# kkoutini/PaSST

Measured on AMD Instinct MI355X. Metric: clips/s (10s@32k) fwd+bwd passt_s, higher is better.
Workload: dtype bf16; 1 GPU; passt_s_swa_p16_128_ap476 train step (mel front end + mixup + fwd + BCE + bwd + adamw), 768/12/12, 474 tokens (s_patchout_t=40,f=4), random-init weights; global_batch=64, per_gpu_batch=64, parallelism=dp1, gemm_launch=persistent, 256 workgroups, input=waveform (B,1,320000) f32 resident in HBM

## Files before the change

### include/passt_amd.h

```cpp
#ifndef PASST_AMD_H
#define PASST_AMD_H

#include <stdint.h>

#ifdef __cplusplus
extern "C" {
#endif

#define PA_ABI_VERSION 6

enum { PA_F32 = 0, PA_BF16 = 1 };

enum {
    PA_OK = 0,
    PA_EINVAL = -1,
    PA_EUNSUPPORTED = -2,
    PA_ELAUNCH = -3,
    PA_ECOMM = -4
};

int pa_abi_version(void);
const char* pa_error_string(int code);
const char* pa_last_hip_error(void);

// ... 103 lines not shown
    int32_t ldolp;
    void* out_lp2;
    int32_t ldolp2;
    int32_t split_k;
    int32_t tune;
    float* colsum_out;
    float* colsum_ws;
    int32_t colsum_accumulate;
    int32_t reserved;
    int32_t colscale_n;
    float colscale;
} pa_gemm_args;
#define PA_GEMM_BLOCKED_PRE 0x100
#define PA_GEMM_NO_PERSIST 0x400
#define PA_GEMM_EPILOGUE_V3 0x1000
#define PA_GEMM_COLSUM_DEFER 0x2000
int pa_gemm_blocked_pre_ok(int M, int N, int K);
int64_t pa_gemm_blocked_pre_elems(int M, int N);
int64_t pa_gemm_colsum_ws_floats(int M, int N);
int pa_gemm_nt(const pa_gemm_args* a, void* stream);
int pa_gemm_nt_splitk_plan(int M, int N, int K, int epilogue, int dtype);
int64_t pa_gemm_nt_splitk_ws_floats(int M, int N, int K, int epilogue, int dtype);
int pa_gemm_nt_splitk(const pa_gemm_args* a, float* ws, int64_t ws_floats, void* stream);
int pa_gemm_nt_rowscale(const pa_gemm_args* a, const float* rowscale, void* stream);
int pa_gemm_nt_splitk_rowscale(const pa_gemm_args* a, const float* rowscale, float* ws, int64_t ws_floats, void* stream);
int pa_gemm_tn(const pa_gemm_args* a, void* stream);
#define PA_TN_BATCH_MAX 4
#ifndef PA_TN_STEP_ROWS
#define PA_TN_STEP_ROWS 48
#endif
int pa_gemm_tn_step_rows(void);
int pa_gemm_tn_batched(const pa_gemm_args* a, int n, void* stream);
int pa_gemm_tn_batched_plan(const pa_gemm_args* a, int n, int n_long, int long_steps, void* stream);
int pa_gather_rows(const void* in, const int32_t* idx, int n_idx, int64_t row_bytes, void* out, void* stream);
int pa_scatter_rows(const void* in, const int32_t* idx, int n_idx, int64_t row_bytes, void* out, void* stream);
int pa_tail_inject(const float* rows, const int32_t* idx, int n_idx, const float* add0, const float* add1, float* dx,
                   void* dx_lp, int dtype, int M, int D, void* stream);
int pa_zero2d(void* ptr, int64_t pitch_bytes, int64_t width_bytes, int64_t rows, void* stream);
int pa_reduce_partials(const float* partial, int splits, int64_t n, float* out, int accumulate,
                       void* stream);
#define PA_REDUCE_BATCH_MAX 12
#define PA_REDUCE_SLABS 0
#define PA_REDUCE_ROWS 1
typedef struct pa_reduce_desc {
    const float* partial;
    float* out;
    int64_t n;
    int32_t splits;
    int32_t accumulate;
    int64_t pitch;
    int32_t mode;
    int32_t reserved;
} pa_reduce_desc;
int pa_reduce_partials_batched(const pa_reduce_desc* d, int n, void* stream);
int pa_gemm_last_colsum_rows(void);
int pa_rowsum(const void* in, int dtype, int R, int C, int ld, float* out, int accumulate,
              void* stream);
int64_t pa_colsum_ws_floats(int R, int C);
int pa_colsum(const void* in, int dtype, int R, int C, int ld, float* out, int accumulate, float* ws,
              void* stream);
int pa_colsum_f32(const float* in, int R, int C, int ld, float* out, int accumulate, void* stream);

#define PA_ATTN_Q_PRESCALED 1
#define PA_ATTN_BWD_TWO_PASS 2
#define PA_ATTN_BWD_SINGLE_PASS 4
#define PA_ATTN_BWD_SINGLE_PASS_W16 8
// ... 138 lines not shown
```

### passt_amd/_lib.py

```python
import ctypes as C
import os

_HERE = os.path.dirname(os.path.abspath(__file__))
LIB_PATH = os.path.join(_HERE, "libpasst_amd.so")
LIB_PATH = os.environ.get("PASST_AMD_LIB", LIB_PATH)

PA_F32, PA_BF16 = 0, 1
EPI_STORE, EPI_GELU, EPI_RESID, EPI_DGELU, EPI_PARTIAL = 0, 1, 2, 3, 4

vp, i32, i64, f32 = C.c_void_p, C.c_int32, C.c_int64, C.c_float


class MelParams(C.Structure):
    _fields_ = [("n_fft", i32), ("hop", i32), ("n_mels", i32), ("n_frames", i32),
                ("preemph", f32), ("mel_low", f32), ("inv_mel_delta", f32), ("log_eps", f32),
                ("out_add", f32), ("out_scale", f32),
                ("fmask_start", i32), ("fmask_end", i32), ("tmask_start", i32), ("tmask_end", i32)]


class MelClipParams(C.Structure):
    _fields_ = [("mel_low", f32), ("inv_mel_delta", f32),
                ("fmask_start", i32), ("fmask_end", i32), ("tmask_start", i32), ("tmask_end", i32)]


# ... 29 lines not shown
    "pa_mel_frontend_fwd_varlen": (i32, [vp, i32, i32, vp, vp, vp, vp, vp, i32, f32, C.POINTER(MelParams), vp]),
    "pa_mel_frontend_bwd": (i32, [vp, i32, i32, vp, vp, vp, vp, vp, vp, i64, C.POINTER(MelParams), vp]),
    "pa_mel_frontend_bwd_varlen": (i32, [vp, i32, i32, vp, vp, vp, vp, vp, i32, vp, vp, i64, C.POINTER(MelParams), vp]),
    "pa_mel_frontend_fwd_varlen_aug": (i32, [vp, i32, i32, vp, vp, vp, vp, vp, i32, f32, C.POINTER(MelParams), vp, vp]),
    "pa_mel_frontend_bwd_varlen_aug": (i32, [vp, i32, i32, vp, vp, vp, vp, vp, i32, vp, vp, i64, C.POINTER(MelParams), vp, vp]),
    "pa_convert_f32": (i32, [vp, vp, i64, i32, vp]),
    "pa_convert_f32_rowscale": (i32, [vp, vp, vp, i32, i32, i32, vp]),
    "pa_convert_to_f32": (i32, [vp, i32, vp, i64, vp]),
    "pa_transpose": (i32, [vp, i32, i32, i32, i32, vp, i32, i32, vp]),
    "pa_stage_weights": (i32, [vp, i32, i32, i32, vp]),
    "pa_layernorm_fwd": (i32, [vp, vp, vp, vp, i32, vp, vp, i32, i32, f32, vp]),
    "pa_layernorm_bwd_ws_floats": (i64, [i32, i32]),
    "pa_layernorm_bwd": (i32, [vp, i32, vp, vp, vp, vp, vp, vp, vp, vp, vp, vp, i32, vp, i32, i32, vp]),
    "pa_layernorm_bwd_rows": (i32, [i32]),
    "pa_layernorm_bwd_partial": (i32, [vp, i32, vp, vp, vp, vp, vp, vp, vp, vp, i32, i32, vp]),
    "pa_layernorm_bwd2": (i32, [vp, i32, vp, vp, vp, vp, vp, vp, vp, vp, vp, vp, vp, i32, vp, i32, i32, vp]),
    "pa_layernorm_bwd2_partial": (i32, [vp, i32, vp, vp, vp, vp, vp, vp, vp, vp, vp, i32, i32, vp]),
    "pa_layernorm_bwd_rowscale": (i32, [vp, i32, vp, vp, vp, vp, vp, vp, vp, vp, vp, vp, vp, vp, i32, vp, i32, i32, vp]),
    "pa_layernorm_bwd_partial_rowscale": (i32, [vp, i32, vp, vp, vp, vp, vp, vp, vp, vp, vp, vp, i32, i32, vp]),
    "pa_tail_inject": (i32, [vp, vp, i32, vp, vp, vp, vp, i32, i32, i32, vp]),
    "pa_gemm_last_colsum_rows": (i32, []),
    "pa_gemm_colsum_ws_floats": (i64, [i32, i32]),
    "pa_gemm_blocked_pre_ok": (i32, [i32, i32, i32]),
    "pa_gemm_blocked_pre_elems": (i64, [i32, i32]),
    "pa_gemm_nt": (i32, [C.POINTER(GemmArgs), vp]),
    "pa_gemm_nt_splitk_plan": (i32, [i32, i32, i32, i32, i32]),
    "pa_gemm_nt_splitk_ws_floats": (i64, [i32, i32, i32, i32, i32]),
    "pa_gemm_nt_splitk": (i32, [C.POINTER(GemmArgs), vp, i64, vp]),
    "pa_gemm_nt_rowscale": (i32, [C.POINTER(GemmArgs), vp, vp]),
    "pa_gemm_nt_splitk_rowscale": (i32, [C.POINTER(GemmArgs), vp, vp, i64, vp]),
    "pa_gemm_tn": (i32, [C.POINTER(GemmArgs), vp]),
    "pa_gemm_tn_batched": (i32, [C.POINTER(GemmArgs), i32, vp]),
    "pa_gemm_tn_batched_plan": (i32, [C.POINTER(GemmArgs), i32, i32, i32, vp]),
    "pa_gemm_tn_step_rows": (i32, []),
    "pa_reduce_partials_batched": (i32, [C.POINTER(ReduceDesc), i32, vp]),
    "pa_colsum_ws_floats": (i64, [i32, i32]),
    "pa_colsum": (i32, [vp, i32, i32, i32, i32, vp, i32, vp, vp]),
    "pa_reduce_partials": (i32, [vp, i32, i64, vp, i32, vp]),
    "pa_rowsum": (i32, [vp, i32, i32, i32, i32, vp, i32, vp]),
    "pa_colsum_f32": (i32, [vp, i32, i32, i32, vp, i32, vp]),
    "pa_attention_fwd": (i32, [vp, i32, vp, i32, vp, i32, i32, i32, i32, f32, i32, i32, vp]),
    "pa_attention_fwd_varlen": (i32, [vp, i32, vp, i32, vp, vp, i32, i32, i32, i32, f32, i32, i32, vp]),
    "pa_attention_probs": (i32, [vp, i32, vp, vp, vp, vp, i32, i32, i32, i32, i32, f32, i32, i32, vp]),
    "pa_attention_probs_grad": (i32, [vp, i32, vp, vp, i32, i32, vp, vp, vp, i32, i32, i32, i32, i32, i32, f32, i32, i32, vp]),
    "pa_attention_rollout_ws_floats": (i64, [i64, i32, i32, i32, i32, i32]),
    "pa_attention_rollout": (i32, [vp, i32, vp, vp, i32, i32, vp, vp, vp, vp, i64, i32, i32, i32, i32, i32, i32, i32, f32, f32, f32, f32,
                                   i32, i32, vp]),
    "pa_attention_bwd_ws_floats": (i64, [i32, i32, i32]),
    "pa_attention_bwd": (i32, [vp, i32, vp, vp, i32, vp, vp, vp, i32, i32, i32, i32, i32, f32, i32, i32, vp]),
    "pa_attention_bwd_varlen_ws_floats": (i64, [i64, i32, i32, i32]),
    "pa_attention_bwd_varlen": (i32, [vp, i32, vp, vp, i32, vp, vp, vp, i32, vp, i32, i32, i32, i32, f32, i32, i32, vp]),
    "pa_gather_rows": (i32, [vp, vp, i32, i64, vp, vp]),
    "pa_scatter_rows": (i32, [vp, vp, i32, i64, vp, vp]),
    "pa_zero2d": (i32, [vp, i64, i64, i64, vp]),
    "pa_patch_gather": (i32, [vp, i32, i32, i32, vp, vp, i32, i32, i32, i32, vp, i32, vp]),
    "pa_patch_pos_table": (i32, [vp, vp, i32, vp, i32, vp, vp, i32, i32, i32, vp, vp, vp, vp, vp, i32, i32, vp]),
    "pa_patch_gather_varlen": (i32, [vp, i32, i32, i32, vp, vp, vp, i32, i32, i32, i32, vp, i32, vp]),
    "pa_patch_pos_table_varlen": (i32, [vp, vp, i32, vp, i32, vp, vp, i32, i32, vp, vp, vp, vp, vp]),
    "pa_patch_input_bwd_varlen": (i32, [vp, i32, vp, i32, i32, i32, i32, i32, i32, vp, vp]),
    "pa_patch_bwd_varlen": (i32, [vp, i32, i32, vp, i32, i32, i32, vp, vp, vp, vp, vp, vp, i32, vp]),
    "pa_patch_input_bwd_rows": (i32, [vp, i32, i32, vp, i32, i32, i32, i32, i32, i32, i32, vp, vp]),
    "pa_patch_bwd_rows": (i32, [vp, i32, i32, vp, vp, vp, i32, i32, i32, i32, vp, vp, vp, vp, vp, vp, i32, vp]),
    "pa_patch_bwd": (i32, [vp, i32, i32, i32, vp, vp, i32, i32, i32, i32, vp, vp, vp, vp, vp, vp, vp, i32, vp, i32, vp]),
    "pa_patch_input_bwd_ws_ints": (i64, [i32, i32, i32, i32, i32]),
    "pa_patch_input_bwd": (i32, [vp, i32, i32, i32, vp, vp, i32, i32, i32, i32, i32, vp, vp, vp]),
    "pa_head_pre_fwd": (i32, [vp, i32, i32, i32, vp, vp, f32, vp, vp, f32, vp, vp, vp, vp]),
# ... 104 lines not shown
```

### passt_amd/csrc/gemm.hip

```cpp
#include <algorithm>
#include <cstring>
#include <type_traits>

#include "pa_mma.h"

namespace pa {

static constexpr int NT_GROUP_M = 4;
static constexpr int BM = 128, BN = 128, KB = 128;
static constexpr int TILE_BYTES = BM * KB;
static constexpr int GEMM_LDS = 2 * 2 * TILE_BYTES;

#ifdef PA_PROBE
__device__ unsigned long long* g_probe_buf = nullptr;
static constexpr int PROBE_SLOTS = 512;
#define PA_PROBE_STAMP(cond, idx)                                                                             \
    do {                                                                                                      \
        if ((cond) && (wave & 3) == 0 && lane == 0 && (idx) < PROBE_SLOTS)                                    \
            ((unsigned long long*)(smem + G::LDS))[(wave >> 2) * PROBE_SLOTS + (idx)] = __builtin_amdgcn_s_memtime(); \
    } while (0)
#define PA_PROBE_FLAG(a, bit) (((a).reserved >> (bit)) & 1)
#define PA_PROBE_STAMP_TN(cond, idx)                                                                          \
    do {                                                                                                      \
        if ((cond) && (wave & 3) == 0 && lane == 0 && (idx) < PROBE_SLOTS)                                    \
            ((unsigned long long*)(smem + TN_LDS))[(wave >> 2) * PROBE_SLOTS + (idx)] = __builtin_amdgcn_s_memtime(); \
    } while (0)
#else
#define PA_PROBE_STAMP(cond, idx) do {} while (0)
#define PA_PROBE_STAMP_TN(cond, idx) do {} while (0)
#define PA_PROBE_FLAG(a, bit) 0
#endif


static constexpr int SLAB_BYTES = 32 * 68 * 4;

static int finish_gemm_colsum(const pa_gemm_args& a, int rows, hipStream_t st);

template <int EPI, int TM> __host__ __device__ constexpr int aux_depth() {
    return EPI == PA_EPI_DGELU ? TM : (EPI == PA_EPI_RESID ? (TM <= 3 ? TM : 2) : 0);
}

template <int EPI>
__device__ __forceinline__ void load_bias8(const pa_gemm_args& a, int n0, int wc, int lane, float (&bias8)[8]) {
    const int ncol = n0 + wc * 64 + (lane & 7) * 8;
#pragma unroll
    for (int e = 0; e < 8; ++e) bias8[e] = 0.f;
    if constexpr (EPI != PA_EPI_PARTIAL && EPI != PA_EPI_DGELU) {
        if (a.bias && ncol < a.N) {
            const f32x4 lo = *(const f32x4*)(a.bias + ncol), hi = *(const f32x4*)(a.bias + ncol + 4);
#pragma unroll
            for (int e = 0; e < 4; ++e) { bias8[e] = lo[e]; bias8[4 + e] = hi[e]; }
        }
    }
}

template <typename T, int EPI, int TM = 2, bool RS = false>
__device__ __forceinline__ void gemm_epilogue(const pa_gemm_args& a, f32x16 (&acc)[TM][2], float* slab, int m0,
                                              int n0, int split, int wr, int wc, int lane, const float (&bias8)[8],
                                              int colsum_row = 0, const float* rowscale = nullptr) {
    static_assert(!RS || EPI == PA_EPI_RESID, "row factors: the residual epilogue only");
    const int erow = lane >> 3, ecol = (lane & 7) * 8;
    const int ncol = n0 + wc * 64 + ecol;
    const bool colok = ncol < a.N;
// ... 1385 lines not shown
            }
#pragma unroll
            for (int i = 0; i < 2; ++i)
#pragma unroll
                for (int j = 0; j < 2; ++j) mma32<T>(acc[i][j], fa[i], fb[j]);
        }
    }
    __syncthreads();
    const float nobias[8] = {0.f, 0.f, 0.f, 0.f, 0.f, 0.f, 0.f, 0.f};
    gemm_epilogue<T, PA_EPI_PARTIAL, 2>(a, acc, (float*)(smem + wave * SLAB_BYTES), m0, n0, blockIdx.y, wr, wc, lane, nobias);
}

__device__ __forceinline__ int tn2_swz(int row, int c) { return row * 512 + ((c ^ ((row & 3) << 2)) << 4); }

__device__ __forceinline__ bf16x8 tn2_frag(const char* tile, int ms, int cbase, int lane) {
    const int p = lane & 15, g = (lane >> 4) & 1, h = lane >> 5;
    const int r1 = ms * 16 + h * 8 + (p >> 2);
    const int col = cbase + g * 16 + (p & 3) * 4;
    const int within = (col & 7) * 2;
    const bf16x4 lo = lds_tr16(tile + tn2_swz(r1, col >> 3) + within);
    const bf16x4 hi = lds_tr16(tile + tn2_swz(r1 + 4, col >> 3) + within);
    bf16x8 f;
    f[0] = lo[0]; f[1] = lo[1]; f[2] = lo[2]; f[3] = lo[3];
    f[4] = hi[0]; f[5] = hi[1]; f[6] = hi[2]; f[7] = hi[3];
    return f;
}

static constexpr int TN_ROWS = PA_TN_STEP_ROWS;
static constexpr int TN_STAGES = 3;
static constexpr int TN_OP_BYTES = TN_ROWS * 512, TN_STAGE_BYTES = 2 * TN_OP_BYTES;
static constexpr int TN_LDS = TN_STAGES * TN_STAGE_BYTES;
static_assert(TN_ROWS % 16 == 0 && TN_ROWS * 512 % (8 * 1024) == 0, "whole 16-token phases, whole 1 KiB pieces per wave");

__device__ __forceinline__ void gemm_tn_stagger_range(const pa_gemm_args& a, const int tiles_n, const int tile_id, const int st_begin,
                                                      const int nsteps, float* out, const int ldo, float* cs_out) {
    const bool CSUM = cs_out != nullptr && tile_id % tiles_n == 0;
    constexpr int TM = 4, WN = 4, MROWS = TN_ROWS, NPH = MROWS / 16;
    constexpr int OP_BYTES = TN_OP_BYTES, STAGE_BYTES = TN_STAGE_BYTES;
    constexpr int PER = OP_BYTES / 1024 / 8;
    extern __shared__ __attribute__((aligned(16))) char smem[];
    const int tid = threadIdx.x;
    const int lane = tid & 63;
    const int wave = __builtin_amdgcn_readfirstlane(tid >> 6);
    const int wr = wave / WN, wc = wave % WN;
    const int bid = tile_id;
    const int m0 = (bid / tiles_n) * 256, n0 = (bid % tiles_n) * 256;
    const int Mtok = a.K;

    uint32_t voffA[PER], voffB[PER];
    int rowin[PER];
#pragma unroll
    for (int i = 0; i < PER; ++i) {
        const int q = wave * PER + i;
        const int row = q * 2 + (lane >> 5);
        const int pc = lane & 31;
        const int c = pc ^ ((row & 3) << 2);
        rowin[i] = row;
        voffA[i] = (uint32_t)row * (uint32_t)a.lda * 2u + (uint32_t)min(m0 + c * 8, a.M - 8) * 2u;
        voffB[i] = (uint32_t)row * (uint32_t)a.ldb * 2u + (uint32_t)min(n0 + c * 8, a.N - 8) * 2u;
    }
    const char* baseA = (const char*)a.A + (int64_t)st_begin * MROWS * a.lda * 2;
    const char* baseB = (const char*)a.B + (int64_t)st_begin * MROWS * a.ldb * 2;
    auto dma = [&](const bool opB, const char* base, int ld, const uint32_t (&voff)[PER], char* dst, int step) __attribute__((always_inline)) {
        const char* sb = base + (int64_t)step * MROWS * ld * 2;
        const int valid = Mtok - (st_begin + step) * MROWS;
        if (valid >= MROWS) {
            if (opB) {
#pragma unroll
// ... 122 lines not shown
#pragma unroll
                    for (int j = 0; j < 2; ++j) mma32_first<bf16>(acc[i][j], fa[i], fb[j]);
            } else {
#pragma unroll
                for (int i = 0; i < TM; ++i)
#pragma unroll
                    for (int j = 0; j < 2; ++j) mma32<bf16>(acc[i][j], fa[i], fb[j]);
            }
            if (CSUM) asm volatile("s_nop 1\n\tv_mfma_f32_32x32x16_bf16 %0, %1, %2, %0" : "+v"(accb) : "v"(fcs), "v"(ones));
            __builtin_amdgcn_s_setprio(0);
            PA_PROBE_STAMP_TN(t >= 4 && t < 12, ((t - 4) * NPH + ph) * 4 + 2);
            if (ph == NPH - 1 && wr == 0) {
                wait_stage();
                asm volatile("s_waitcnt lgkmcnt(0)" ::: "memory");
            }
            __builtin_amdgcn_sched_barrier(0);
            __builtin_amdgcn_s_barrier();
            PA_PROBE_STAMP_TN(t >= 4 && t < 12, ((t - 4) * NPH + ph) * 4 + 3);
        };
        phase(std::integral_constant<int, 0>{});
        phase(std::integral_constant<int, 1>{});
        phase(std::integral_constant<int, 2>{});
        if constexpr (NPH == 4) phase(std::integral_constant<int, 3>{});
        static_assert(NPH == 3 || NPH == 4, "three or four 16-token phases per stage");
        slot = slot1;
    }
    if (wr == 0) __builtin_amdgcn_s_barrier();
#ifdef PA_PROBE
    __syncthreads();
    if (g_probe_buf && blockIdx.x < 8)
        for (int i = tid; i < 2 * PROBE_SLOTS; i += 512)
            g_probe_buf[(size_t)blockIdx.x * 2 * PROBE_SLOTS + i] = ((unsigned long long*)(smem + TN_LDS))[i];
#endif
    {
        pa_gemm_args e = a;
        e.out_f32 = out;
        e.ldo32 = ldo;
        gemm_epilogue_f32_direct<PA_EPI_PARTIAL, TM>(e, acc, nullptr, m0, n0, 0, wr, wc, lane);
    }
    if (CSUM) {
        if ((lane & 31) == 0) {
            float* dst = cs_out;
#pragma unroll
            for (int r = 0; r < 16; ++r) {
                const int m = m0 + wr * 128 + wc * 32 + acc_row(r, lane);
                if (m < a.M) dst[m] = accb[r];
            }
        }
    }
}

__device__ __forceinline__ void gemm_tn_stagger_item(const pa_gemm_args& a, const int tiles_n, const int tile_id, const int split,
                                                     const int steps_per_split) {
    const int steps_total = (a.K + TN_ROWS - 1) / TN_ROWS;
    const int st_begin = split * steps_per_split;
    const int nsteps = min(steps_total, st_begin + steps_per_split) - st_begin;
    gemm_tn_stagger_range(a, tiles_n, tile_id, st_begin, nsteps, a.out_f32 + (int64_t)split * a.M * a.ldo32, a.ldo32,
                          a.colsum_ws ? a.colsum_ws + (int64_t)split * a.M : nullptr);
}

__global__ __launch_bounds__(512) void gemm_tn_stagger_kernel(const pa_gemm_args a, const int tiles_n, const int nwg,
                                                              const int steps_per_split) {
    gemm_tn_stagger_item(a, tiles_n, xcd_swizzle(blockIdx.x, nwg), blockIdx.y, steps_per_split);
}

struct TnBatch {
    pa_gemm_args a[PA_TN_BATCH_MAX];
    int32_t first[PA_TN_BATCH_MAX + 1];
    int32_t tiles_n[PA_TN_BATCH_MAX], nwg[PA_TN_BATCH_MAX], per[PA_TN_BATCH_MAX];
    int32_t tfirst[PA_TN_BATCH_MAX + 1];
    int32_t n, order;
};
__global__ __launch_bounds__(512) void gemm_tn_stagger_batched_kernel(const TnBatch b) {
    int p = 0, t, split;
    if (b.order == 1) {
        const int logical = xcd_swizzle(blockIdx.x, b.first[b.n]);
        const int tiles_all = b.tfirst[b.n];
        split = logical / tiles_all;
        t = logical - split * tiles_all;
        while (p + 1 < b.n && t >= b.tfirst[p + 1]) ++p;
        t -= b.tfirst[p];
    } else {
        while (p + 1 < b.n && (int)blockIdx.x >= b.first[p + 1]) ++p;
        const int item = blockIdx.x - b.first[p];
        split = item / b.nwg[p];
        t = xcd_swizzle(item - split * b.nwg[p], b.nwg[p]);
    }
    gemm_tn_stagger_item(b.a[p], b.tiles_n[p], t, split, b.per[p]);
}

struct TnPlan {
    pa_gemm_args a[PA_TN_BATCH_MAX];
    int32_t tiles_n[PA_TN_BATCH_MAX];
    int32_t tfirst[PA_TN_BATCH_MAX + 1];
    int32_t n, n_long, long_steps, steps;
};
__global__ __launch_bounds__(512) void gemm_tn_stagger_plan_kernel(const TnPlan b) {
    const int tiles_all = b.tfirst[b.n], nlong = tiles_all * b.n_long;
    int g, t;
    if ((int)blockIdx.x < nlong) {
        const int logical = xcd_swizzle(blockIdx.x, nlong);
        g = logical / tiles_all;
        t = logical - g * tiles_all;
    } else {
        g = b.n_long;
        t = xcd_swizzle(blockIdx.x - nlong, tiles_all);
    }
    int p = 0;
    while (p + 1 < b.n && t >= b.tfirst[p + 1]) ++p;
    t -= b.tfirst[p];
    const pa_gemm_args& a = b.a[p];
    const int st_begin = g * b.long_steps;
    const int nsteps = g < b.n_long ? b.long_steps : b.steps - st_begin;
    gemm_tn_stagger_range(a, b.tiles_n[p], t, st_begin, nsteps, a.out_f32 + (int64_t)g * a.M * a.ldo32, a.ldo32,
                          a.colsum_ws ? a.colsum_ws + (int64_t)g * a.M : nullptr);
}

static int launch_gemm_tn_stagger(const pa_gemm_args& a, hipStream_t st) {
#ifdef PA_PROBE
    constexpr int LDS = TN_LDS + 2 * PROBE_SLOTS * 8;
#else
    constexpr int LDS = TN_LDS;
#endif
    const int tiles_m = (int)cdiv(a.M, 256), tiles_n = (int)cdiv(a.N, 256);
    const int nwg = tiles_m * tiles_n;
    const int steps = (int)cdiv(a.K, TN_ROWS);
    const int per = (int)cdiv(steps, a.split_k);
    static signed char lds_attr[64] = {0};
    (void)lds_attr_on_this_device((const void*)gemm_tn_stagger_kernel, LDS, lds_attr);
    hipLaunchKernelGGL(gemm_tn_stagger_kernel, dim3(nwg, a.split_k), dim3(512), LDS, st, a, tiles_n, nwg, per);
    return check_launch();
}

template <typename T>
static int launch_gemm_tn(const pa_gemm_args& a, hipStream_t st) {
    const int tiles_m = (int)cdiv(a.M, BM), tiles_n = (int)cdiv(a.N, BN);
    const int nwg = tiles_m * tiles_n;
    const int steps = (int)cdiv(a.K, TNGeom<T>::MROWS);
    const int per = (int)cdiv(steps, a.split_k);
    static signed char lds_attr[64] = {0};
    (void)lds_attr_on_this_device((const void*)gemm_tn_kernel<T>, GEMM_LDS, lds_attr);
    hipLaunchKernelGGL((gemm_tn_kernel<T>), dim3(nwg, a.split_k), dim3(256), GEMM_LDS, st, a, tiles_n, nwg, per);
    return check_launch();
}

template <typename T>
__global__ __launch_bounds__(256) void colsum_stage1_kernel(const T* __restrict__ in, int R, int C, int ld,
                                                            float* __restrict__ part, int rows_per_block) {
// ... 529 lines not shown
    TnPlan plan;
    TnPlan* pb = &plan;
    int64_t tiles = 0;
    for (int p = 0; p < n; ++p) {
        const pa_gemm_args& x = a[p];
        if (!x.A || !x.B || !x.out_f32 || x.M <= 0 || x.N <= 0 || x.K <= 0 || x.split_k != n_long + 1) return PA_EINVAL;
        if (x.dtype != PA_BF16 || x.epilogue != PA_EPI_PARTIAL) return PA_EUNSUPPORTED;
        if ((x.lda * 2) % 16 || (x.ldb * 2) % 16 || x.ldo32 % 4 || x.M < 8 || x.N < 8 || x.N % 8 || x.M % 8) return PA_EUNSUPPORTED;
        if (x.K != a[0].K) return PA_EUNSUPPORTED;
        pb->a[p] = x;
        pb->tiles_n[p] = (int)cdiv(x.N, 256);
        pb->tfirst[p] = (int)tiles;
        tiles += cdiv(x.M, 256) * pb->tiles_n[p];
    }
    const int steps = (int)cdiv(a[0].K, TN_ROWS);
    if ((int64_t)n_long * long_steps >= steps) return PA_EINVAL;
    if (tiles * (n_long + 1) > INT32_MAX) return PA_EUNSUPPORTED;
    pb->tfirst[n] = (int)tiles;
    pb->n = n;
    pb->n_long = n_long;
    pb->long_steps = long_steps;
    pb->steps = steps;
#ifdef PA_PROBE
    constexpr int LDS = TN_LDS + 2 * PROBE_SLOTS * 8;
#else
    constexpr int LDS = TN_LDS;
#endif
    static signed char lds_attr[64] = {0};
    (void)lds_attr_on_this_device((const void*)gemm_tn_stagger_plan_kernel, LDS, lds_attr);
    hipLaunchKernelGGL(gemm_tn_stagger_plan_kernel, dim3((unsigned)(tiles * (n_long + 1))), dim3(512), LDS, (hipStream_t)stream, plan);
    return check_launch();
}

namespace pa {
struct ReduceBatch {
    pa_reduce_desc d[PA_REDUCE_BATCH_MAX];
    int32_t n;
};
__global__ __launch_bounds__(256) void reduce_partials_batched_kernel(const ReduceBatch b) {
    const pa_reduce_desc& d = b.d[blockIdx.y];
    if (d.mode == PA_REDUCE_ROWS) {
        __shared__ float red[16][17];
        const int cx = threadIdx.x & 15, ry = threadIdx.x >> 4;
        for (int64_t c0 = (int64_t)blockIdx.x * 16; c0 < d.n; c0 += (int64_t)gridDim.x * 16) {
            const int64_t k = c0 + cx;
            float s = 0.f, s1 = 0.f, s2 = 0.f, s3 = 0.f;
            if (k < d.n) {
                int r = ry;
                for (; r + 48 < d.splits; r += 64) {
                    s += d.partial[(int64_t)r * d.pitch + k];
                    s1 += d.partial[(int64_t)(r + 16) * d.pitch + k];
                    s2 += d.partial[(int64_t)(r + 32) * d.pitch + k];
                    s3 += d.partial[(int64_t)(r + 48) * d.pitch + k];
                }
                for (; r < d.splits; r += 16) s += d.partial[(int64_t)r * d.pitch + k];
            }
            red[ry][cx] = (s + s1) + (s2 + s3);
            __syncthreads();
            if (ry == 0 && k < d.n) {
                float t = 0.f;
#pragma unroll
                for (int y = 0; y < 16; ++y) t += red[y][cx];
                d.out[k] = (d.accumulate ? d.out[k] : 0.f) + t;
            }
            __syncthreads();
        }
// ... 69 lines not shown
    return check_launch();
}

namespace pa {
__global__ __launch_bounds__(256) void zero2d_kernel(char* __restrict__ p, int64_t pitch, int64_t w16, int64_t rows) {
    const int64_t n = rows * w16, stride = (int64_t)gridDim.x * blockDim.x;
    for (int64_t i = (int64_t)blockIdx.x * blockDim.x + threadIdx.x; i < n; i += stride) {
        const int64_t r = i / w16, c = i - r * w16;
        *(f32x4*)(p + r * pitch + c * 16) = f32x4{0.f, 0.f, 0.f, 0.f};
    }
}
}

extern "C" int pa_zero2d(void* ptr, int64_t pitch_bytes, int64_t width_bytes, int64_t rows, void* stream) {
    if (!ptr || pitch_bytes < width_bytes || width_bytes <= 0 || rows <= 0) return PA_EINVAL;
    if (pitch_bytes != width_bytes && ((uintptr_t)ptr | pitch_bytes | width_bytes) % 16 == 0) {
        const int64_t w16 = width_bytes / 16;
        const int blocks = (int)std::min<int64_t>(cdiv(rows * w16, 256), 8192);
        hipLaunchKernelGGL(zero2d_kernel, dim3(blocks), dim3(256), 0, (hipStream_t)stream, (char*)ptr, pitch_bytes, w16, rows);
        return check_launch();
    }
    hipError_t e = pitch_bytes == width_bytes
                       ? hipMemsetAsync(ptr, 0, (size_t)(width_bytes * rows), (hipStream_t)stream)
                       : hipMemset2DAsync(ptr, (size_t)pitch_bytes, 0, (size_t)width_bytes, (size_t)rows, (hipStream_t)stream);
    return e == hipSuccess ? PA_OK : set_hip_error(e);
}

#ifdef PA_PROBE
extern "C" int pa_probe_set_buffer(void* dev_buf) {
    unsigned long long* p = (unsigned long long*)dev_buf;
    hipError_t e = hipMemcpyToSymbol(HIP_SYMBOL(pa::g_probe_buf), &p, sizeof(p));
    return e == hipSuccess ? PA_OK : pa::set_hip_error(e);
}
#endif
```

### passt_amd/ops.py

```python
import collections
import ctypes as C
import functools
import threading
import os

import numpy as np
import torch

from . import _lib
from ._lib import (GEMM_BLOCKED_PRE, EPI_DGELU, EPI_GELU, EPI_PARTIAL, EPI_RESID, EPI_STORE, PA_BF16, PA_F32,
                   GemmArgs, MelParams, check)

TORCH_DTYPE = {PA_F32: torch.float32, PA_BF16: torch.bfloat16}
PA_DTYPE = {torch.float32: PA_F32, torch.bfloat16: PA_BF16}


class _CallState(threading.local):
    dev = None
    gemm_flags = 0


_call = _CallState()


# ... 606 lines not shown
        score = eff - 0.003 * S
        if score > best_score:
            best, best_score = S, score
    return best


_SPLITS_CACHE = {}
_FORCE_SLICES = int(os.environ.get("PASST_AMD_WGRAD_SLICES", "0"))


def pick_batched_splits(probs, slots=256):
    key = (tuple(probs), slots)
    hit = _SPLITS_CACHE.get(key)
    if hit is None:
        hit = _SPLITS_CACHE[key] = _pick_batched_splits(list(probs), slots)
        if _FORCE_SLICES:
            hit = _SPLITS_CACHE[key] = [max(1, min(_FORCE_SLICES, st)) for _, st in probs]
    return hit


def _pick_batched_splits(probs, slots=256):
    best, best_cost = None, None
    for L in range(max(p[1] for p in probs), 3, -1):
        S = [max(1, min(64, -(-st // L))) for _, st in probs]
        items = sum(t * s_ for (t, _), s_ in zip(probs, S))
        per = max(-(-st // s_) for (_, st), s_ in zip(probs, S))
        cost = -(-items // slots) * (per + 4) * 1.2 + items * 0.05
        if best_cost is None or cost < best_cost - 1e-9:
            best, best_cost = S, cost
    return best if best is not None else [1] * len(probs)


_PLAN_CACHE = {}
WGRAD_PLAN_DEFAULT = "long_short"
_SHORT_ITEM_COST = 1.25
_PLAN_MIN_GAIN = 0.04
_FORCE_UNIFORM = os.environ.get("PASST_AMD_WGRAD_PLAN", WGRAD_PLAN_DEFAULT) == "uniform" or _FORCE_SLICES > 0


def pick_batched_plan(probs, slots=256):
    if _FORCE_UNIFORM:
        return 0, 0, pick_batched_splits(probs, slots)
    key = (tuple(probs), slots)
    hit = _PLAN_CACHE.get(key)
    if hit is None:
        hit = _PLAN_CACHE[key] = _pick_batched_plan(list(probs), slots)
    return hit


def _uniform_cost(probs, S, slots=256):
    items = sum(t * s_ for (t, _), s_ in zip(probs, S))
    per = max(-(-st // s_) for (_, st), s_ in zip(probs, S))
    return -(-items // slots) * (per + 4) * 1.2 + items * 0.05


def _long_short_cost(tiles, steps, a, L, slots=256):
    import heapq
    free = [0.0] * slots
    end = 0.0
    for steps_item, count, k in ((L, a * tiles, 1.0), (steps - a * L, tiles, _SHORT_ITEM_COST)):
        dur = (steps_item + 4) * 1.2 * k
        for _ in range(count):
            t = free[0] + dur
            heapq.heapreplace(free, t)
            end = max(end, t)
    return end + tiles * (a + 1) * 0.05


def _pick_batched_plan(probs, slots=256):
    S = _pick_batched_splits(probs, slots)
    steps = probs[0][1]
    tiles = sum(t for t, _ in probs)
    if any(st != steps for _, st in probs) or sum(t * s_ for (t, _), s_ in zip(probs, S)) <= slots:
        return 0, 0, S
    best, best_cost = (0, 0, S), _uniform_cost(probs, S, slots)
    for a in (1, 2):
        for L in range((steps - 1) // a, -(-steps // (a + 1)) - 1, -1):
            cost = _long_short_cost(tiles, steps, a, L, slots)
            if cost < best_cost - 1e-9:
                best, best_cost = (a, L, [a + 1] * len(probs)), cost
    return best if best_cost < (1.0 - _PLAN_MIN_GAIN) * _uniform_cost(probs, S, slots) else (0, 0, S)


def wgrad_batched_ws_floats(splits, shapes):
    return sum(S * N * (K + (1 if has_db else 0)) for S, (N, K, has_db) in zip(splits, shapes))


def wgrad_tn(dY, X, out_f32, dtype, accumulate=False, partial_ws=None, db=None):
    Mtok, N = dY.shape
    K = X.shape[1]
    if dtype == PA_BF16 and GEMM_TUNE != 1:
        tiles = ((N + 255) // 256) * ((K + 255) // 256)
        S = pick_split_k_slots(tiles, (Mtok + tn_step_rows() - 1) // tn_step_rows())
    else:
        tiles = ((N + 127) // 128) * ((K + 127) // 128)
        mrows = 64 if dtype == PA_BF16 else 32
        S = pick_split_k(tiles, (Mtok + mrows - 1) // mrows)
    assert db is None or wgrad_tn_fuses_bias(dtype)
    need = S * N * K + (S * N if db is not None else 0)
    if partial_ws is None or partial_ws.numel() < need:
        partial_ws = torch.empty(need, device=dY.device, dtype=torch.float32)
    part = partial_ws[:S * N * K].view(S, N, K)
    a = GemmArgs()
    a.dtype, a.epilogue = dtype, EPI_PARTIAL
    a.M, a.N, a.K = N, K, Mtok
    a.lda, a.ldb = dY.stride(0), X.stride(0)
    a.A, a.B = _p(dY, dtype, True), _p(X, dtype, True)
    a.out_f32, a.ldo32 = _p(part), K
    a.split_k = S
    a.tune = GEMM_TUNE
    bpart = partial_ws[S * N * K:need] if db is not None else None
    a.colsum_ws = _p(bpart)
    lib = _lib.load()
    ev0 = ev1 = None
    if GEMM_PROFILE is not None:
        ev0, ev1 = torch.cuda.Event(enable_timing=True), torch.cuda.Event(enable_timing=True)
        ev0.record()
    check(lib.pa_gemm_tn(C.byref(a), _stream()), "pa_gemm_tn")
    check(lib.pa_reduce_partials(_p(part), S, N * K, _p(out_f32), int(accumulate), _stream()), "pa_reduce_partials")
    if db is not None:
        check(lib.pa_reduce_partials(_p(bpart), S, N, _p(db, torch.float32), int(accumulate), _stream()), "pa_reduce_partials")
    if ev0 is not None:
        ev1.record()
        GEMM_PROFILE.setdefault("wgrad_tn", []).append((ev0, ev1, 2.0 * N * K * Mtok))
    return partial_ws


def wgrad_tn_fuses_bias(dtype):
    return dtype == PA_BF16 and GEMM_TUNE != 1


def wgrad_tn_batched(problems, dtype, partial_ws=None, row_jobs=None, plan=None):
    from ._lib import ReduceDesc
    assert dtype == PA_BF16 and 1 <= len(problems) <= 4
    problems = [tuple(p) + (None,) * (5 - len(p)) for p in problems]
    metas = []
    for dY, X, out, acc, db in problems:
        Mtok, N = dY.shape
        metas.append((Mtok, N, X.shape[1]))
    shapes = [(((N + 255) // 256) * ((K + 255) // 256), (Mtok + tn_step_rows() - 1) // tn_step_rows()) for Mtok, N, K in metas]
    if plan is None:
        n_long, long_steps, splits = pick_batched_plan(shapes)
    elif plan[0] == 0:
        n_long, long_steps, splits = 0, 0, pick_batched_splits(shapes)
    else:
        n_long, long_steps = plan
        splits = [n_long + 1] * len(problems)
    need = wgrad_batched_ws_floats(splits, [(m[1], m[2], p[4] is not None) for m, p in zip(metas, problems)])
    if partial_ws is None or partial_ws.numel() < need:
        partial_ws = torch.empty(need, device=problems[0][0].device, dtype=torch.float32)
    row_jobs = row_jobs or []
    nred = len(problems) + sum(1 for p in problems if p[4] is not None) + len(row_jobs)
    args = (GemmArgs * len(problems))()
    red = (ReduceDesc * nred)()
    off, flops, k = 0, 0.0, len(problems)
    for a, r, (dY, X, out, acc, db), (Mtok, N, K), S in zip(args, red, problems, metas, splits):
        part = partial_ws[off:off + S * N * K]
        off += S * N * K
        a.dtype, a.epilogue = dtype, EPI_PARTIAL
        a.M, a.N, a.K = N, K, Mtok
        a.lda, a.ldb = dY.stride(0), X.stride(0)
        a.A, a.B = _p(dY, dtype, True), _p(X, dtype, True)
        a.out_f32, a.ldo32 = _p(part), K
        a.split_k, a.tune = S, TN_BATCH_ORDER
        r.partial, r.out, r.n, r.splits, r.accumulate = _p(part), _p(out, torch.float32), N * K, S, int(acc)
        if db is not None:
            bpart = partial_ws[off:off + S * N]
            off += S * N
            a.colsum_ws = _p(bpart)
            rb = red[k]
            k += 1
            rb.partial, rb.out, rb.n, rb.splits, rb.accumulate = _p(bpart), _p(db, torch.float32), N, S, int(acc)
        flops += 2.0 * N * K * Mtok
    for part_rows, rows, pitch, n, out in row_jobs:
        rb = red[k]
        k += 1
        rb.partial, rb.out, rb.n, rb.splits, rb.accumulate = _p(part_rows, torch.float32, True), _p(out, torch.float32), n, rows, 0
        rb.pitch, rb.mode = pitch, _lib.REDUCE_ROWS
    lib = _lib.load()
    ev0 = ev1 = None
    if GEMM_PROFILE is not None:
        ev0, ev1 = torch.cuda.Event(enable_timing=True), torch.cuda.Event(enable_timing=True)
        ev0.record()
    if n_long:
        check(lib.pa_gemm_tn_batched_plan(args, len(problems), n_long, long_steps, _stream()), "pa_gemm_tn_batched_plan")
    else:
        check(lib.pa_gemm_tn_batched(args, len(problems), _stream()), "pa_gemm_tn_batched")
    for lo in range(0, nred, REDUCE_BATCH_MAX):
        n = min(REDUCE_BATCH_MAX, nred - lo)
        check(lib.pa_reduce_partials_batched(C.cast(C.byref(red, lo * C.sizeof(ReduceDesc)), C.POINTER(ReduceDesc)), n, _stream()),
              "pa_reduce_partials_batched")
    if ev0 is not None:
        ev1.record()
        GEMM_PROFILE.setdefault("wgrad_tn", []).append((ev0, ev1, flops))
    return partial_ws


REDUCE_BATCH_MAX = 12


def colsum(x, out_f32, accumulate=False):
    R, Cc = x.shape
    lib = _lib.load()
    ws = torch.empty(lib.pa_colsum_ws_floats(R, Cc), device=x.device, dtype=torch.float32)
    check(lib.pa_colsum(_p(x, None, True), PA_DTYPE[x.dtype], R, Cc, x.stride(0), _p(out_f32, torch.float32), int(accumulate), _p(ws),
                        _stream()), "pa_colsum")


def rowsum(x, out_f32, ncols=None, accumulate=False):
    R, Cc = x.shape
    check(_lib.load().pa_rowsum(_p(x, None, True), PA_DTYPE[x.dtype], R, Cc if ncols is None else ncols, x.stride(0),
                                _p(out_f32), int(accumulate), _stream()), "pa_rowsum")


def colsum_f32(x, out_f32, accumulate=False):
    R, Cc = x.shape
    check(_lib.load().pa_colsum_f32(_p(x, torch.float32, True), R, Cc, x.stride(0), _p(out_f32, torch.float32), int(accumulate), _stream()),
# ... 609 lines not shown
```

Baseline: 2859 clips/s.

## Add persistent dealt work-queue scheduler for batched weight-gradient TN GEMM

New measurement: 2870 clips/s (median of 6 runs). Within noise of the previous version (+0.4%).

```diff
diff --git a/include/passt_amd.h b/include/passt_amd.h
--- a/include/passt_amd.h
+++ b/include/passt_amd.h
@@ -159,6 +159,8 @@
 int pa_gemm_tn_step_rows(void);
 int pa_gemm_tn_batched(const pa_gemm_args* a, int n, void* stream);
 int pa_gemm_tn_batched_plan(const pa_gemm_args* a, int n, int n_long, int long_steps, void* stream);
+int64_t pa_gemm_tn_dealt_ws_bytes(void);
+int pa_gemm_tn_batched_dealt(const pa_gemm_args* a, int n, int n_long, int long_steps, int n_short, void* ws, void* stream);
 int pa_gather_rows(const void* in, const int32_t* idx, int n_idx, int64_t row_bytes, void* out, void* stream);
 int pa_scatter_rows(const void* in, const int32_t* idx, int n_idx, int64_t row_bytes, void* out, void* stream);
 int pa_tail_inject(const float* rows, const int32_t* idx, int n_idx, const float* add0, const float* add1, float* dx,
diff --git a/passt_amd/_lib.py b/passt_amd/_lib.py
--- a/passt_amd/_lib.py
+++ b/passt_amd/_lib.py
@@ -85,6 +85,8 @@
     "pa_gemm_tn": (i32, [C.POINTER(GemmArgs), vp]),
     "pa_gemm_tn_batched": (i32, [C.POINTER(GemmArgs), i32, vp]),
     "pa_gemm_tn_batched_plan": (i32, [C.POINTER(GemmArgs), i32, i32, i32, vp]),
+    "pa_gemm_tn_dealt_ws_bytes": (i64, []),
+    "pa_gemm_tn_batched_dealt": (i32, [C.POINTER(GemmArgs), i32, i32, i32, i32, vp, vp]),
     "pa_gemm_tn_step_rows": (i32, []),
     "pa_reduce_partials_batched": (i32, [C.POINTER(ReduceDesc), i32, vp]),
     "pa_colsum_ws_floats": (i64, [i32, i32]),
diff --git a/passt_amd/csrc/gemm.hip b/passt_amd/csrc/gemm.hip
--- a/passt_amd/csrc/gemm.hip
+++ b/passt_amd/csrc/gemm.hip
@@ -25,10 +25,25 @@
         if ((cond) && (wave & 3) == 0 && lane == 0 && (idx) < PROBE_SLOTS)                                    \
             ((unsigned long long*)(smem + TN_LDS))[(wave >> 2) * PROBE_SLOTS + (idx)] = __builtin_amdgcn_s_memtime(); \
     } while (0)
+__device__ unsigned long long* g_probe_items = nullptr;
+#define PA_PROBE_ITEM_BEGIN() const unsigned long long probe_t0 = __builtin_amdgcn_s_memrealtime()
+#define PA_PROBE_ITEM_END(item, slice, seq)                                                                   \
+    do {                                                                                                      \
+        if (g_probe_items && threadIdx.x == 0) {                                                              \
+            unsigned long long* r = g_probe_items + (size_t)(item) * 4;                                       \
+            r[0] = probe_t0;                                                                                  \
+            r[1] = __builtin_amdgcn_s_memrealtime();                                                          \
+            r[2] = ((unsigned long long)__builtin_amdgcn_s_getreg(4 | (31 << 11)) << 32) |                   \
+                   (unsigned)__builtin_amdgcn_s_getreg(20 | (31 << 11));                                      \
+            r[3] = ((unsigned long long)blockIdx.x << 32) | ((unsigned)(slice) << 16) | (unsigned)(seq);      \
+        }                                                                                                     \
+    } while (0)
 #else
 #define PA_PROBE_STAMP(cond, idx) do {} while (0)
 #define PA_PROBE_STAMP_TN(cond, idx) do {} while (0)
 #define PA_PROBE_FLAG(a, bit) 0
+#define PA_PROBE_ITEM_BEGIN() do {} while (0)
+#define PA_PROBE_ITEM_END(item, slice, seq) do {} while (0)
 #endif
 
 
@@ -1480,8 +1495,12 @@
 static constexpr int TN_LDS = TN_STAGES * TN_STAGE_BYTES;
 static_assert(TN_ROWS % 16 == 0 && TN_ROWS * 512 % (8 * 1024) == 0, "whole 16-token phases, whole 1 KiB pieces per wave");
 
+struct tn_no_seam {
+    __device__ __forceinline__ void operator()() const {}
+};
+template <typename Seam = tn_no_seam>
 __device__ __forceinline__ void gemm_tn_stagger_range(const pa_gemm_args& a, const int tiles_n, const int tile_id, const int st_begin,
-                                                      const int nsteps, float* out, const int ldo, float* cs_out) {
+                                                      const int nsteps, float* out, const int ldo, float* cs_out, Seam seam = Seam{}) {
     const bool CSUM = cs_out != nullptr && tile_id % tiles_n == 0;
     constexpr int TM = 4, WN = 4, MROWS = TN_ROWS, NPH = MROWS / 16;
     constexpr int OP_BYTES = TN_OP_BYTES, STAGE_BYTES = TN_STAGE_BYTES;
@@ -1670,6 +1689,7 @@
         for (int i = tid; i < 2 * PROBE_SLOTS; i += 512)
             g_probe_buf[(size_t)blockIdx.x * 2 * PROBE_SLOTS + i] = ((unsigned long long*)(smem + TN_LDS))[i];
 #endif
+    seam();
     {
         pa_gemm_args e = a;
         e.out_f32 = out;
@@ -1734,6 +1754,7 @@
     int32_t n, n_long, long_steps, steps;
 };
 __global__ __launch_bounds__(512) void gemm_tn_stagger_plan_kernel(const TnPlan b) {
+    PA_PROBE_ITEM_BEGIN();
     const int tiles_all = b.tfirst[b.n], nlong = tiles_all * b.n_long;
     int g, t;
     if ((int)blockIdx.x < nlong) {
@@ -1752,6 +1773,75 @@
     const int nsteps = g < b.n_long ? b.long_steps : b.steps - st_begin;
     gemm_tn_stagger_range(a, b.tiles_n[p], t, st_begin, nsteps, a.out_f32 + (int64_t)g * a.M * a.ldo32, a.ldo32,
                           a.colsum_ws ? a.colsum_ws + (int64_t)g * a.M : nullptr);
+    PA_PROBE_ITEM_END(blockIdx.x, g, 0);
+}
+
+struct TnDealt {
+    pa_gemm_args a[PA_TN_BATCH_MAX];
+    int32_t tiles_n[PA_TN_BATCH_MAX];
+    int32_t tfirst[PA_TN_BATCH_MAX + 1];
+    int32_t n, n_long, long_steps, n_short, short_steps, steps;
+    uint32_t* tickets;
+};
+static constexpr int TN_DEALT_QUEUES = 8;
+__global__ __launch_bounds__(512) void gemm_tn_stagger_dealt_kernel(const TnDealt b, const int lds_bytes) {
+    extern __shared__ __attribute__((aligned(16))) char smem[];
+    int* const s_item = (int*)(smem + lds_bytes - 16);
+    const int tiles_all = b.tfirst[b.n], nlong = tiles_all * b.n_long, nshort = tiles_all * b.n_short;
+    const int home = blockIdx.x & (TN_DEALT_QUEUES - 1);
+    const int lq = nlong >> 3, lr = nlong & 7, sq = nshort >> 3, sr = nshort & 7;
+    auto entry = [&](const int x, const int i) -> int {
+        const int lcnt = lq + (x < lr), scnt = sq + (x < sr);
+        if (i < lcnt) return (x < lr ? x * (lq + 1) : lr * (lq + 1) + (x - lr) * lq) + i;
+        if (i - lcnt < scnt) return nlong + (x < sr ? x * (sq + 1) : sr * (sq + 1) + (x - sr) * sq) + (i - lcnt);
+        return -1;
+    };
+    auto homes = [&](const int x) -> int { return (int)(gridDim.x >> 3) + (x < (int)(gridDim.x & 7)); };
+    auto take = [&]() {
+        const int lane = threadIdx.x & 63, x = (home + lane) & (TN_DEALT_QUEUES - 1);
+        const unsigned seen = lane < TN_DEALT_QUEUES ? __hip_atomic_load(b.tickets + x, __ATOMIC_RELAXED, __HIP_MEMORY_SCOPE_AGENT) : 0u;
+        const bool left = lane < TN_DEALT_QUEUES && seen < 0x40000000u && (int)seen + homes(x) < lq + (x < lr) + sq + (x < sr);
+        unsigned long long cand = __ballot(left);
+        if (lane == 0) {
+            int item = -1;
+            while (cand != 0 && item < 0) {
+                const int r = __ffsll((long long)cand) - 1, xr = (home + r) & (TN_DEALT_QUEUES - 1);
+                cand &= cand - 1;
+                const unsigned v = __hip_atomic_fetch_add(b.tickets + xr, 1u, __ATOMIC_RELAXED, __HIP_MEMORY_SCOPE_AGENT);
+                item = entry(xr, (int)min(v + (unsigned)homes(xr), 0x7fffffffu));
+            }
+            *s_item = item;
+        }
+    };
+    int item = entry(home, (int)(blockIdx.x >> 3));
+    if (item < 0) {
+        if (threadIdx.x < 64) take();
+        __syncthreads();
+        item = *s_item;
+    }
+    [[maybe_unused]] int seq = 0;
+    while (item >= 0) {
+        PA_PROBE_ITEM_BEGIN();
+        const int logical = item < nlong ? item : item - nlong;
+        const int q = logical / tiles_all;
+        int t = logical - q * tiles_all;
+        const int g = item < nlong ? q : b.n_long + q;
+        int p = 0;
+        while (p + 1 < b.n && t >= b.tfirst[p + 1]) ++p;
+        t -= b.tfirst[p];
+        const pa_gemm_args& a = b.a[p];
+        const int st_begin = item < nlong ? q * b.long_steps : b.n_long * b.long_steps + q * b.short_steps;
+        const int nsteps = item < nlong ? b.long_steps : min(b.short_steps, b.steps - st_begin);
+        int next = -1;
+        gemm_tn_stagger_range(a, b.tiles_n[p], t, st_begin, nsteps, a.out_f32 + (int64_t)g * a.M * a.ldo32, a.ldo32,
+                              a.colsum_ws ? a.colsum_ws + (int64_t)g * a.M : nullptr, [&]() {
+                                  if (threadIdx.x < 64) take();
+                                  __syncthreads();
+                                  next = *s_item;
+                              });
+        PA_PROBE_ITEM_END(item, g, seq++);
+        item = next;
+    }
 }
 
 static int launch_gemm_tn_stagger(const pa_gemm_args& a, hipStream_t st) {
@@ -2347,6 +2437,58 @@
     return check_launch();
 }
 
+extern "C" int64_t pa_gemm_tn_dealt_ws_bytes(void) { return (TN_DEALT_QUEUES * (int64_t)sizeof(uint32_t) + 15) / 16 * 16; }
+
+extern "C" int pa_gemm_tn_batched_dealt(const pa_gemm_args* a, int n, int n_long, int long_steps, int n_short, void* ws, void* stream) {
+    if (!a || !ws || n < 1 || n > PA_TN_BATCH_MAX || n_long < 1 || long_steps < 1 || n_short < 1) return PA_EINVAL;
+    if ((uintptr_t)ws % 4) return PA_EINVAL;
+    TnDealt plan;
+    TnDealt* pb = &plan;
+    int64_t tiles = 0;
+    for (int p = 0; p < n; ++p) {
+        const pa_gemm_args& x = a[p];
+        if (!x.A || !x.B || !x.out_f32 || x.M <= 0 || x.N <= 0 || x.K <= 0 || x.split_k != n_long + n_short) return PA_EINVAL;
+        if (x.dtype != PA_BF16 || x.epilogue != PA_EPI_PARTIAL) return PA_EUNSUPPORTED;
+        if ((x.lda * 2) % 16 || (x.ldb * 2) % 16 || x.ldo32 % 4 || x.M < 8 || x.N < 8 || x.N % 8 || x.M % 8) return PA_EUNSUPPORTED;
+        if (x.K != a[0].K) return PA_EUNSUPPORTED;
+        pb->a[p] = x;
+        pb->tiles_n[p] = (int)cdiv(x.N, 256);
+        pb->tfirst[p] = (int)tiles;
+        tiles += cdiv(x.M, 256) * pb->tiles_n[p];
+    }
+    const int steps = (int)cdiv(a[0].K, TN_ROWS);
+    if ((int64_t)n_long * long_steps >= steps) return PA_EINVAL;
+    const int rest = steps - n_long * long_steps, short_steps = (int)cdiv(rest, n_short);
+    if (rest - (int64_t)(n_short - 1) * short_steps < 1) return PA_EINVAL;
+    if (tiles * (n_long + n_short) > INT32_MAX / 2) return PA_EUNSUPPORTED;
+    pb->tfirst[n] = (int)tiles;
+    pb->n = n;
+    pb->n_long = n_long;
+    pb->long_steps = long_steps;
+    pb->n_short = n_short;
+    pb->short_steps = short_steps;
+    pb->steps = steps;
+    pb->tickets = (uint32_t*)ws;
+#ifdef PA_PROBE
+    constexpr int LDS = TN_LDS + 2 * PROBE_SLOTS * 8 + 16;
+#else
+    constexpr int LDS = TN_LDS + 16;
+#endif
+    static int cus[64] = {0};
+    int dev = 0;
+    if (hipGetDevice(&dev) != hipSuccess || dev < 0 || dev >= 64) return set_hip_error(hipErrorInvalidDevice);
+    if (cus[dev] == 0) {
+        int c = 0;
+        cus[dev] = (hipDeviceGetAttribute(&c, hipDeviceAttributeMultiprocessorCount, dev) == hipSuccess && c > 0) ? c : 256;
+    }
+    static signed char lds_attr[64] = {0};
+    (void)lds_attr_on_this_device((const void*)gemm_tn_stagger_dealt_kernel, LDS, lds_attr);
+    const hipError_t e = hipMemsetAsync(ws, 0, (size_t)pa_gemm_tn_dealt_ws_bytes(), (hipStream_t)stream);
+    if (e != hipSuccess) return set_hip_error(e);
+    hipLaunchKernelGGL(gemm_tn_stagger_dealt_kernel, dim3((unsigned)cus[dev]), dim3(512), LDS, (hipStream_t)stream, plan, LDS);
+    return check_launch();
+}
+
 namespace pa {
 struct ReduceBatch {
     pa_reduce_desc d[PA_REDUCE_BATCH_MAX];
@@ -2482,4 +2624,9 @@
     hipError_t e = hipMemcpyToSymbol(HIP_SYMBOL(pa::g_probe_buf), &p, sizeof(p));
     return e == hipSuccess ? PA_OK : pa::set_hip_error(e);
 }
+extern "C" int pa_probe_set_items(void* dev_buf) {
+    unsigned long long* p = (unsigned long long*)dev_buf;
+    hipError_t e = hipMemcpyToSymbol(HIP_SYMBOL(pa::g_probe_items), &p, sizeof(p));
+    return e == hipSuccess ? PA_OK : pa::set_hip_error(e);
+}
 #endif
diff --git a/passt_amd/ops.py b/passt_amd/ops.py
--- a/passt_amd/ops.py
+++ b/passt_amd/ops.py
@@ -662,7 +662,7 @@
 
 
 _PLAN_CACHE = {}
-WGRAD_PLAN_DEFAULT = "long_short"
+WGRAD_PLAN_DEFAULT = "dealt"
 _SHORT_ITEM_COST = 1.25
 _PLAN_MIN_GAIN = 0.04
 _FORCE_UNIFORM = os.environ.get("PASST_AMD_WGRAD_PLAN", WGRAD_PLAN_DEFAULT) == "uniform" or _FORCE_SLICES > 0
@@ -710,6 +710,74 @@
             if cost < best_cost - 1e-9:
                 best, best_cost = (a, L, [a + 1] * len(probs)), cost
     return best if best_cost < (1.0 - _PLAN_MIN_GAIN) * _uniform_cost(probs, S, slots) else (0, 0, S)
+
+
+_WGRAD_PLAN = os.environ.get("PASST_AMD_WGRAD_PLAN", WGRAD_PLAN_DEFAULT)
+_FORCE_DEALT = tuple(int(v) for v in os.environ.get("PASST_AMD_WGRAD_DEALT", "").split(",") if v) or None
+_DEALT_SEAM_US = 1.5
+_DEALT_MAX_SLABS = 3
+_DEALT_CACHE = {}
+_DEALT_WS = {}
+
+
+def _dealt_cost(tiles, steps, a, L, s, slots=256):
+    import heapq
+    rest = steps - a * L
+    per = -(-rest // s)
+    free = [0.0] * slots
+    end = 0.0
+    for steps_item, count in ((L, a * tiles), (per, (s - 1) * tiles), (rest - (s - 1) * per, tiles)):
+        dur = (steps_item + 4) * 1.2
+        for _ in range(count):
+            t = free[0] + dur + (_DEALT_SEAM_US if free[0] > 0.0 else 0.0)
+            heapq.heapreplace(free, t)
+            end = max(end, t)
+    return end + tiles * (a + s) * 0.05
+
+
+def _pick_dealt_plan(probs, slots=256):
+    steps = probs[0][1]
+    tiles = sum(t for t, _ in probs)
+    if any(st != steps for _, st in probs):
+        return None
+    n_long, L, S = _pick_batched_plan(probs, slots)
+    if not n_long and sum(t * s_ for (t, _), s_ in zip(probs, S)) <= slots:
+        return None
+    today = _long_short_cost(tiles, steps, n_long, L, slots) if n_long else _uniform_cost(probs, S, slots)
+    best, best_cost = None, today
+    for a in (1, 2):
+        for s in range(1, _DEALT_MAX_SLABS - a + 1):
+            for L in range((steps - 1) // a, 0, -1):
+                rest = steps - a * L
+                per = -(-rest // s)
+                if rest - (s - 1) * per < 1 or per > L:
+                    continue
+                cost = _dealt_cost(tiles, steps, a, L, s, slots)
+                if cost < best_cost - 1e-9:
+                    best, best_cost = (a, L, s), cost
+    return best
+
+
+def pick_dealt_plan(probs, slots=256):
+    if _FORCE_DEALT:
+        a, L, s = _FORCE_DEALT
+        steps = probs[0][1]
+        rest = steps - a * L
+        ok = all(st == steps for _, st in probs) and rest >= 1 and rest - (s - 1) * -(-rest // s) >= 1
+        return _FORCE_DEALT if ok else None
+    key = (tuple(probs), slots)
+    if key not in _DEALT_CACHE:
+        _DEALT_CACHE[key] = _pick_dealt_plan(list(probs), slots)
+    return _DEALT_CACHE[key]
+
+
+def dealt_ws(device):
+    dev = torch.device(device)
+    key = (dev.index, torch.cuda.current_stream(dev).cuda_stream)
+    ws = _DEALT_WS.get(key)
+    if ws is None:
+        ws = _DEALT_WS[key] = torch.zeros(_lib.load().pa_gemm_tn_dealt_ws_bytes(), device=dev, dtype=torch.uint8)
+    return ws
 
 
 def wgrad_batched_ws_floats(splits, shapes):
@@ -769,13 +837,20 @@
         Mtok, N = dY.shape
         metas.append((Mtok, N, X.shape[1]))
     shapes = [(((N + 255) // 256) * ((K + 255) // 256), (Mtok + tn_step_rows() - 1) // tn_step_rows()) for Mtok, N, K in metas]
+    n_short = 0
     if plan is None:
-        n_long, long_steps, splits = pick_batched_plan(shapes)
+        dealt = pick_dealt_plan(shapes) if _WGRAD_PLAN == "dealt" else None
+        if dealt is not None:
+            n_long, long_steps, n_short = dealt
+            splits = [n_long + n_short] * len(problems)
+        else:
+            n_long, long_steps, splits = pick_batched_plan(shapes)
     elif plan[0] == 0:
         n_long, long_steps, splits = 0, 0, pick_batched_splits(shapes)
     else:
-        n_long, long_steps = plan
-        splits = [n_long + 1] * len(problems)
+        n_long, long_steps = plan[:2]
+        n_short = plan[2] if len(plan) > 2 else 0
+        splits = [n_long + max(1, n_short)] * len(problems)
     need = wgrad_batched_ws_floats(splits, [(m[1], m[2], p[4] is not None) for m, p in zip(metas, problems)])
     if partial_ws is None or partial_ws.numel() < need:
         partial_ws = torch.empty(need, device=problems[0][0].device, dtype=torch.float32)
@@ -812,7 +887,10 @@
     if GEMM_PROFILE is not None:
         ev0, ev1 = torch.cuda.Event(enable_timing=True), torch.cuda.Event(enable_timing=True)
         ev0.record()
-    if n_long:
+    if n_short:
+        check(lib.pa_gemm_tn_batched_dealt(args, len(problems), n_long, long_steps, n_short, _p(dealt_ws(problems[0][0].device)),
+                                           _stream()), "pa_gemm_tn_batched_dealt")
+    elif n_long:
         check(lib.pa_gemm_tn_batched_plan(args, len(problems), n_long, long_steps, _stream()), "pa_gemm_tn_batched_plan")
     else:
         check(lib.pa_gemm_tn_batched(args, len(problems), _stream()), "pa_gemm_tn_batched")
```
